# schmrlng/MotionPlanning.jl

Hardware: AMD Instinct MI355X
Metric: edges checked/sec + r-disc queries/sec, FMT* N=1e6 R^6, 1/2/4/8 MI355X (higher is better)
Workload: dtype f64

## Files before the change

### motionplanning.jl_amd/csrc/kernels_order.hip

```cpp
#include "mpfmt_internal.h"
#include <algorithm>

#define ORD_ID(k) ((k) & 0x03ffffffu)
#define ORD_COL(k) (((k) >> 26) & 15u)
#define ORD_THREADS 512
#define ORD_WAVES 8
#define ORD_COLS 16
#define ORD_NB 128
#define ORD_STG 2560
#define ORD_PRE 5
#define ORD_WAVES_EU 8
static_assert(ORD_STG >= MPFMT_ORD_MAXDEG, "a column the host lets through must fit the staging area");
static_assert(ORD_COLS * ORD_NB == ORD_THREADS * 4, "the segmented scan gives every thread four buckets");
static_assert(ORD_PRE * ORD_THREADS >= ORD_STG && ORD_STG % 32 == 0 && ORD_STG < 65536, "the prefetched records cover what the staging area holds; positions fit 16 bits");

struct ord_hdr {
    int32_t k[ORD_COLS];
    int32_t cb[ORD_COLS + 4];
    long long out[ORD_COLS];
    int32_t ho[ORD_COLS];
    int32_t n, pad_[3];
};
struct ord_shared {
    uint32_t cnt[ORD_COLS][ORD_NB / 2];
    uint32_t cur[ORD_COLS][ORD_NB / 2];
    ord_hdr h[2];
    int32_t g1, pcount, nextk, pad_;
    uint32_t bits[ORD_STG / 32];
};

__device__ __forceinline__ void lds_barrier()
{
    asm volatile("s_waitcnt lgkmcnt(0)\n\ts_barrier" ::: "memory");
}

struct ord_args {
    const uint32_t* qkey;
    const double* qd2;
    long long qcap;
    const int32_t* qlen;
    const int64_t* degs;
    int64_t tile_begin, tile_end;
    const int64_t* colptr;
    const int32_t* perm;
    const int32_t* iperm;
    int32_t* rowval;
    double* nzval;
    int32_t* rowpos;
    uint32_t bucket_mul;
    const int32_t* spec_fail;
    unsigned long long* mask;
    const int64_t* nnz_dev;
    uint4* pend_items; int64_t pend_wcap; int32_t* pend_cnt; int32_t* pend_over;
    int64_t* deg_clear;
    int rec_bits;
    int32_t* qctr;
};

__global__ __launch_bounds__(ORD_THREADS) __attribute__((amdgpu_waves_per_eu(ORD_WAVES_EU, ORD_WAVES_EU))) void k_order_logs(ord_args a)
{
    if (a.spec_fail && *a.spec_fail) return;
    extern __shared__ __attribute__((aligned(16))) char ord_smem[];
    double* const stage_d2 = reinterpret_cast<double*>(ord_smem);
    uint32_t* const stage_key = reinterpret_cast<uint32_t*>(ord_smem + ORD_STG * 8);
    ord_shared& sh = *reinterpret_cast<ord_shared*>(ord_smem + ORD_STG * 12);
    const int tid = threadIdx.x, lane = tid & 63;
    const int wave = __builtin_amdgcn_readfirstlane(tid >> 6);
    const int64_t nq = (a.tile_end - a.tile_begin) * 4;
    auto bucket = [&](uint32_t id) -> int { return a.bucket_mul ? min(ORD_NB - 1, (int)__umulhi(id, a.bucket_mul)) : (int)(id & (ORD_NB - 1)); };
    if (a.rec_bits && blockIdx.x == 0 && tid == 0) {
        const int64_t nnz = *a.nnz_dev;
        if (nnz & 63) atomicAnd(&a.mask[nnz >> 6], (1ull << (nnz & 63)) - 1ull);
    }

    int hk = 0, ho = -1, hln = 0;
    long long hout = 0;
    auto hdr_fetch1 = [&](int64_t qi) {
        hk = 0; ho = -1; hln = 0;
        if (qi >= nq) return;
        if (tid < ORD_COLS) {
            const int64_t sp = a.tile_begin * 64 + qi * ORD_COLS + tid;
            ho = a.perm[sp];
            hk = (int)a.degs[sp];
            if (a.deg_clear && ho >= 0) a.deg_clear[ho] = 0;
        } else if (tid == 64) {
            hln = (int)min((long long)a.qlen[qi], a.qcap);
        }
    };
    auto hdr_fetch2 = [&]() { hout = (tid < ORD_COLS && ho >= 0) ? a.colptr[ho] : 0; };
    auto hdr_publish = [&](int hb) {
        ord_hdr& H = sh.h[hb];
        if (tid < 64) {
            const int k = (tid < ORD_COLS && ho >= 0) ? hk : 0;
            int inc = k;
            inc += __builtin_amdgcn_update_dpp(0, inc, 0x111, 0xf, 0xf, true);
            inc += __builtin_amdgcn_update_dpp(0, inc, 0x112, 0xf, 0xf, true);
            inc += __builtin_amdgcn_update_dpp(0, inc, 0x114, 0xf, 0xf, true);
            inc += __builtin_amdgcn_update_dpp(0, inc, 0x118, 0xf, 0xf, true);
            if (tid < ORD_COLS) { H.k[tid] = k; H.cb[tid + 1] = inc; H.ho[tid] = ho; }
            if (tid == 0) H.cb[0] = 0;
        } else if (tid == 64) {
            H.n = hln;
        }
    };
    uint32_t pk[ORD_PRE];
    double pd[ORD_PRE];
    auto rec_fetch_n = [&](int total, int64_t qi) {
        const __amdgpu_buffer_rsrc_t rk = __builtin_amdgcn_make_buffer_rsrc(const_cast<uint32_t*>(a.qkey + (qi < nq ? qi : 0) * a.qcap), 0, total * 4, 0x00020000);
#pragma unroll
        for (int u = 0; u < ORD_PRE; ++u) pk[u] = __builtin_amdgcn_raw_buffer_load_b32(rk, tid * 4, u * ORD_THREADS * 4, 0);
    };
    auto rec_fetch = [&](const ord_hdr& H, int64_t qi) { rec_fetch_n((qi < nq) ? H.n : 0, qi); };
    typedef uint32_t ord_u32x2 __attribute__((ext_vector_type(2)));
    auto d2_fetch = [&](int total, int64_t qi) {
        const long long base = (qi < nq ? qi : 0) * a.qcap;
        const __amdgpu_buffer_rsrc_t rd = __builtin_amdgcn_make_buffer_rsrc(const_cast<double*>(a.qd2 + base), 0, total * 8, 0x00020000);
#pragma unroll
        for (int u = 0; u < ORD_PRE; ++u) {
            const ord_u32x2 v = __builtin_amdgcn_raw_buffer_load_b64(rd, tid * 8, u * ORD_THREADS * 8, 0);
            pd[u] = __hiloint2double((int)v.y, (int)v.x);
        }
    };

    if (tid == 0) sh.pcount = 0;
    int64_t qi = blockIdx.x;
    int64_t qn = qi + gridDim.x;
    const int xcd = (int)(blockIdx.x & 7u);
    int hb = 0;
    hdr_fetch1(qi);
    hdr_fetch2();
    hdr_publish(0);
    if (tid < ORD_COLS) sh.h[0].out[tid] = hout;
    lds_barrier();
    rec_fetch(sh.h[0], qi);
    d2_fetch(sh.h[0].n, qi);
    for (; qi < nq; hb ^= 1) {
        const ord_hdr& H = sh.h[hb];
        const int total = H.n;
        const long long lbase = qi * a.qcap;
        hdr_fetch1(qn);
            int g0 = 0;
        bool first = true;
        while (g0 < ORD_COLS) {
            if (tid < 64) {
                const bool ok = tid >= g0 && tid < ORD_COLS && (H.cb[min(tid, ORD_COLS - 1) + 1] - H.cb[g0] <= ORD_STG);
                const unsigned long long m = __ballot(ok);
                if (tid == 0) sh.g1 = g0 + (int)__popcll(m);
            }
            *reinterpret_cast<uint2*>(&sh.cnt[0][tid * 2]) = make_uint2(0u, 0u);
            lds_barrier();
            int g1 = sh.g1;
            const bool skip = g1 == g0;
            if (skip) g1 = g0 + 1;
            const int gb = H.cb[g0];
            auto for_records = [&](auto&& f) {
                if (first) {
#pragma unroll
                    for (int u = 0; u < ORD_PRE; ++u) if (u * ORD_THREADS + tid < total) {
                        uint32_t key = pk[u];
                        asm volatile("" : "+v"(key));
                        f(key, u, u * ORD_THREADS + tid);
                    }
                }
                for (int i = (first ? ORD_PRE * ORD_THREADS : 0) + tid; i < total; i += ORD_THREADS) f(a.qkey[lbase + i], -1, i);
            };
            if (!skip) for_records([&](uint32_t key, int, int) {
                const int col = (int)ORD_COL(key);
                if (col >= g0 && col < g1) { const int bk = bucket(ORD_ID(key)); atomicAdd(&sh.cnt[col][bk >> 1], 1u << ((bk & 1) * 16)); }
            });
            lds_barrier();
            {
                const int col = tid >> 5;
                const uint2 cw = *reinterpret_cast<const uint2*>(&sh.cnt[0][tid * 2]);
                const int c0 = (int)(cw.x & 0xffffu), c1 = (int)(cw.x >> 16), c2 = (int)(cw.y & 0xffffu), c3 = (int)(cw.y >> 16);
                const int tot = c0 + c1 + c2 + c3;
                int inc = tot;
                inc += __builtin_amdgcn_update_dpp(0, inc, 0x111, 0xf, 0xf, true);
                inc += __builtin_amdgcn_update_dpp(0, inc, 0x112, 0xf, 0xf, true);
                inc += __builtin_amdgcn_update_dpp(0, inc, 0x114, 0xf, 0xf, true);
                inc += __builtin_amdgcn_update_dpp(0, inc, 0x118, 0xf, 0xf, true);
                inc += __builtin_amdgcn_update_dpp(0, inc, 0x142, 0xa, 0xf, false);
                const int b0 = min(max(H.cb[col] - gb + inc - tot, 0), ORD_STG);
                const int b1 = min(b0 + c0, ORD_STG), b2 = min(b1 + c1, ORD_STG), b3 = min(b2 + c2, ORD_STG);
                *reinterpret_cast<uint2*>(&sh.cur[0][tid * 2]) = make_uint2((uint32_t)b0 | ((uint32_t)b1 << 16), (uint32_t)b2 | ((uint32_t)b3 << 16));
            }
            lds_barrier();
            if (!skip) for_records([&](uint32_t key, int u, int i) {
                const int col = (int)ORD_COL(key);
                if (col >= g0 && col < g1) {
                    const int bk = bucket(ORD_ID(key));
                    const int pos = (int)((atomicAdd(&sh.cur[col][bk >> 1], 1u << ((bk & 1) * 16)) >> ((bk & 1) * 16)) & 0xffffu);
                    double d2 = 0.0;
                    if (u < 0) d2 = a.qd2[lbase + i];
#pragma unroll
                    for (int v = 0; v < ORD_PRE; ++v) if (u == v) d2 = pd[v];
                    if (pos >= 0 && pos < ORD_STG) { stage_key[pos] = key; stage_d2[pos] = d2; }
                }
            });
            if (a.rec_bits && tid < ORD_STG / 32) sh.bits[tid] = 0xffffffffu;
            lds_barrier();
            if (first) {
                hdr_fetch2();
                hdr_publish(hb ^ 1);
                if (a.qctr && tid == 0) sh.nextk = atomicAdd(&a.qctr[xcd], 1);
                first = false;
            }
            const bool last_range = g1 >= ORD_COLS;
            if (last_range) {
                lds_barrier();
                rec_fetch(sh.h[hb ^ 1], qn);
                d2_fetch(qn < nq ? sh.h[hb ^ 1].n : 0, qn);
            }
            if (!skip) {
                const int nst = min(H.cb[g1] - gb, ORD_STG);
                for (int p0 = 0; p0 < nst; p0 += ORD_THREADS) {
                    const int p = p0 + tid;
                    const bool act = p < nst;
                    if (p0 + wave * 64 >= nst) break;
                    const uint32_t key = act ? stage_key[p] : ((uint32_t)(g1 - 1) << 26);
                    const int col = (int)ORD_COL(key);
                    const uint32_t id = ORD_ID(key);
                    const int bk = bucket(id);
                    const int e = (int)((sh.cur[col][bk >> 1] >> ((bk & 1) * 16)) & 0xffffu), n = (int)((sh.cnt[col][bk >> 1] >> ((bk & 1) * 16)) & 0xffffu);
                    int rk = e - n;
                    if (act) {
                        const int b0 = e - n, bl = e - 1;
                        const uint32_t m0 = ORD_ID(stage_key[b0]), m1 = ORD_ID(stage_key[min(b0 + 1, bl)]), m2 = ORD_ID(stage_key[min(b0 + 2, bl)]),
                                       m3 = ORD_ID(stage_key[min(b0 + 3, bl)]);
                        rk += (int)(m0 < id) + (int)(n > 1 && m1 < id) + (int)(n > 2 && m2 < id) + (int)(n > 3 && m3 < id);
                        for (int m = b0 + 4; m < e; ++m) rk += (ORD_ID(stage_key[m]) < id) ? 1 : 0;
                    }
                    const int rel = rk - (H.cb[col] - gb);
                    const bool valid = act && rel >= 0 && rel < H.k[col];
                    const int64_t o = H.out[col] + rel;
                    int32_t rp = 0;
                    const bool pd_ = valid && a.pend_items && ((key >> 30) & 1u);
                    if ((valid && a.rowpos) || pd_) rp = a.iperm[id];
                    if (valid) {
                        a.rowval[o] = (int32_t)id;
                        a.nzval[o] = sqrt(stage_d2[p]);
                        if (a.rowpos) a.rowpos[o] = rp;
                    }
                    if (a.rec_bits && valid && (key >> 31)) atomicAnd(&sh.bits[rk >> 5], ~(1u << (rk & 31)));
                    if (a.pend_items) {
                        const unsigned long long pm = __ballot(pd_);
                        if (pm) {
                            int base = 0;
                            if (lane == 0) base = atomicAdd(&sh.pcount, (int)__popcll(pm));
                            base = __builtin_amdgcn_readfirstlane(base);
                            if (pd_) {
                                const int pos = base + (int)__builtin_amdgcn_mbcnt_hi((uint32_t)(pm >> 32), __builtin_amdgcn_mbcnt_lo((uint32_t)pm, 0u));
                                if (pos < a.pend_wcap)
                                    a.pend_items[(int64_t)blockIdx.x * a.pend_wcap + pos] =
                                        make_uint4((uint32_t)(uint64_t)o, (uint32_t)((uint64_t)o >> 32), (uint32_t)H.ho[col], (uint32_t)rp);
                            }
                        }
                    }
                }
            }
            lds_barrier();
            if (a.rec_bits) {
                if (!skip) for (int c = g0 + 2 * wave; c < min(g1, g0 + 2 * wave + 2); ++c) {
                    const int k = H.k[c];
                    if (k == 0) continue;
                    const int sb = H.cb[c] - gb;
                    const int64_t o = H.out[c];
                    const int64_t w0 = o >> 6;
                    const int nw = (int)(((o + k - 1) >> 6) - w0) + 1;
                    for (int i = lane; i < nw; i += 64) {
                        const int64_t wd = w0 + i;
                        const int64_t lo_bit = max(wd * 64, o), hi_bit = min(wd * 64 + 64, o + k);
                        const int nb = (int)(hi_bit - lo_bit);
                        const int src = sb + (int)(lo_bit - o);
                        const int wi = src >> 5, sh5 = src & 31;
                        const unsigned long long a0 = sh.bits[wi], a1 = sh.bits[min(wi + 1, ORD_STG / 32 - 1)], a2 = sh.bits[min(wi + 2, ORD_STG / 32 - 1)];
                        unsigned long long val = (a0 | (a1 << 32)) >> sh5;
                        if (sh5) val |= a2 << (64 - sh5);
                        const unsigned long long keep = (nb == 64) ? ~0ull : ((1ull << nb) - 1ull);
                        const int dsh = (int)(lo_bit & 63);
                        const unsigned long long rng = keep << dsh;
                        const unsigned long long w64 = ((val & keep) << dsh) | ~rng;
                        if (w64 != ~0ull) atomicAnd(&a.mask[wd], w64);
                    }
                }
                lds_barrier();
            }
            g0 = g1;
        }
        if (tid < ORD_COLS) sh.h[hb ^ 1].out[tid] = hout;
        qi = qn;
        qn = a.qctr ? 2 * (int64_t)gridDim.x + xcd + 8 * (int64_t)sh.nextk : qn + gridDim.x;
    }
    if (a.pend_items) {
        lds_barrier();
        if (tid == 0) {
            const int c = sh.pcount;
            a.pend_cnt[blockIdx.x] = (int32_t)min((int64_t)c, a.pend_wcap);
            if (c > a.pend_wcap) *a.pend_over = 1;
        }
    }
}

int32_t mpfmt_mask_preset(mpfmt_ctx* ctx, int64_t entries)
{
    int32_t rc;
    const int64_t words = (entries + 63) / 64;
    if ((rc = ctx->graph_free.ensure(ctx, sizeof(uint64_t) * (size_t)(words + 1)))) return rc;
    HIPCHK(ctx, hipMemsetAsync(ctx->graph_free, 0xFF, sizeof(uint64_t) * (size_t)std::max<int64_t>(words, 1), ctx->stream));
    ctx->mask_preset_words = words;
    return MPFMT_OK;
}

int32_t mpfmt_order_logs(mpfmt_ctx* ctx, const int32_t* spec_fail, int64_t mask_entries)
{
    const int64_t nt = ctx->tile_end - ctx->tile_begin;
    int32_t rc;
    ctx->rowpos_valid = false;
    const bool recbits = ctx->bits_in_records;
    const bool pend = ctx->broad_in_drain && !recbits;
    if (recbits) {
        const int64_t words = (std::max<int64_t>(ctx->nnz, mask_entries) + 63) / 64;
        const int64_t words_alloc = (std::max<int64_t>((int64_t)((double)ctx->nnz * 1.02) + 4096, mask_entries) + 63) / 64 + 1;
        if ((rc = ctx->graph_free.ensure(ctx, sizeof(uint64_t) * (size_t)words_alloc))) return rc;
        if (!(ctx->mask_preset_words == words && ctx->nnz > 0))
            HIPCHK(ctx, hipMemsetAsync(ctx->graph_free, ctx->nnz > 0 ? 0xFF : 0, sizeof(uint64_t) * (size_t)std::max<int64_t>(words, 1), ctx->stream));
    }
    ctx->mask_preset_words = -1;
    if (ctx->nnz == 0 || nt <= 0) { if ((rc = mpfmt_side_join(ctx))) return rc; if (recbits) { ctx->graph_swept = true; ctx->sweep_in_order = true; } return MPFMT_OK; }
    const bool want_rowpos = !pend && !recbits;
    if (want_rowpos && (rc = ctx->rowpos.ensure(ctx, sizeof(int32_t) * (size_t)std::max<int64_t>(std::max(ctx->nnz, ctx->nnz_cap), 1)))) return rc;
    const size_t lds = (size_t)ORD_STG * 12 + sizeof(ord_shared);
    HIPCHK(ctx, hipFuncSetAttribute((const void*)k_order_logs, hipFuncAttributeMaxDynamicSharedMemorySize, (int)lds));
    if (ctx->ord_per_cu == 0) {
        int per_cu = 0;
        HIPCHK(ctx, hipOccupancyMaxActiveBlocksPerMultiprocessor(&per_cu, k_order_logs, ORD_THREADS, lds));
        ctx->ord_per_cu = std::max(1, std::min(per_cu, 4));
    }
    unsigned nb = (unsigned)std::min<int64_t>(nt * 4, (int64_t)ctx->num_cus * ctx->ord_per_cu);
    const bool draw = ctx->ord_draw && ctx->ord_ctr && nb >= 8 && (ctx->ord_draw > 1 || ctx->nnz >= (int64_t)1536 * nt * 4);
    if (draw) nb &= ~3u;
    if (pend) {
        const int64_t entries = std::max<int64_t>(ctx->nnz, ctx->nnz_cap);
        ctx->pend_wcap = ctx->debug_small_lists ? 8 : entries * 3 / (2 * (int64_t)nb) + 4096;
        if ((rc = ctx->pend_items.ensure(ctx, sizeof(uint4) * (size_t)ctx->pend_wcap * nb))) return rc;
        if ((rc = ctx->pend_cnt.ensure(ctx, sizeof(int32_t) * (size_t)(nb + 1)))) return rc;
        ctx->pend_over = ctx->pend_cnt + nb;
        HIPCHK(ctx, hipMemsetAsync(ctx->pend_over, 0, sizeof(int32_t), ctx->stream));
    }
    ord_args a{};
    a.qkey = ctx->qkey; a.qd2 = ctx->qd2; a.qcap = ctx->qcap; a.qlen = ctx->qlen; a.degs = ctx->degs;
    a.tile_begin = ctx->tile_begin; a.tile_end = ctx->tile_end; a.colptr = ctx->colptr; a.perm = ctx->perm; a.iperm = ctx->iperm;
    a.rowval = ctx->rowval; a.nzval = ctx->nzval; a.rowpos = want_rowpos ? ctx->rowpos : nullptr;
    a.bucket_mul = ctx->N > 128 ? (uint32_t)((128ull << 32) / (uint64_t)ctx->N) : 0u;
    a.spec_fail = spec_fail;
    a.mask = (unsigned long long*)ctx->graph_free.get(); a.nnz_dev = ctx->colptr + ctx->N;
    a.pend_items = pend ? (uint4*)ctx->pend_items.get() : nullptr; a.pend_wcap = ctx->pend_wcap; a.pend_cnt = ctx->pend_cnt; a.pend_over = ctx->pend_over;
    a.rec_bits = recbits ? 1 : 0;
    a.deg_clear = ctx->world > 1 ? ctx->deg : nullptr;
    a.qctr = draw ? ctx->ord_ctr : nullptr;
    if ((rc = mpfmt_side_join(ctx))) return rc;
    hipLaunchKernelGGL(k_order_logs, dim3(nb), dim3(ORD_THREADS), lds, ctx->stream, a);
    HIPCHK(ctx, hipGetLastError());
    if (pend) ctx->pend_nseg = (int)nb;
    ctx->pend_valid = pend;
    ctx->rowpos_valid = want_rowpos;
    if (recbits) { ctx->graph_swept = true; ctx->sweep_in_order = true; }
    return MPFMT_OK;
}
```

Baseline: 31.07 billion.

## Deepen order-kernel header pipeline to three stages and prefetch keys earlier

```diff
diff --git a/motionplanning.jl_amd/csrc/kernels_order.hip b/motionplanning.jl_amd/csrc/kernels_order.hip
--- a/motionplanning.jl_amd/csrc/kernels_order.hip
+++ b/motionplanning.jl_amd/csrc/kernels_order.hip
@@ -1,5 +1,7 @@
 #include "mpfmt_internal.h"
 #include <algorithm>
+#include <cstdio>
+#include <cstdlib>
 
 #define ORD_ID(k) ((k) & 0x03ffffffu)
 #define ORD_COL(k) (((k) >> 26) & 15u)
@@ -9,6 +11,7 @@
 #define ORD_NB 128
 #define ORD_STG 2560
 #define ORD_PRE 5
+#define ORD_CLK_N 12
 #define ORD_WAVES_EU 8
 static_assert(ORD_STG >= MPFMT_ORD_MAXDEG, "a column the host lets through must fit the staging area");
 static_assert(ORD_COLS * ORD_NB == ORD_THREADS * 4, "the segmented scan gives every thread four buckets");
@@ -24,15 +27,28 @@
 struct ord_shared {
     uint32_t cnt[ORD_COLS][ORD_NB / 2];
     uint32_t cur[ORD_COLS][ORD_NB / 2];
-    ord_hdr h[2];
+    ord_hdr h[3];
     int32_t g1, pcount, nextk, pad_;
     uint32_t bits[ORD_STG / 32];
+#ifdef ORD_CLOCK
+    unsigned long long clk[ORD_CLK_N];
+#endif
 };
+static_assert(ORD_STG * 12 + sizeof(ord_shared) <= 40960, "four workgroups per CU: a quarter of the CU's 160 KB of LDS each");
 
 __device__ __forceinline__ void lds_barrier()
 {
     asm volatile("s_waitcnt lgkmcnt(0)\n\ts_barrier" ::: "memory");
 }
+
+#ifdef ORD_CLOCK
+__device__ unsigned long long ord_clk_dev[4096][ORD_CLK_N];
+#define ORD_CLK(i) do { if (wave == 0) { const unsigned long long t_ = __builtin_readcyclecounter(); if (lane == 0) atomicAdd(&sh.clk[i], t_ - clk_prev); clk_prev = t_; } } while (0)
+#define ORD_CLK_USE5(x) asm volatile("" :: "v"(x[0]), "v"(x[1]), "v"(x[2]), "v"(x[3]), "v"(x[4]))
+#else
+#define ORD_CLK(i) do {} while (0)
+#define ORD_CLK_USE5(x) do {} while (0)
+#endif
 
 struct ord_args {
     const uint32_t* qkey;
@@ -57,7 +73,7 @@
     int32_t* qctr;
 };
 
-__global__ __launch_bounds__(ORD_THREADS) __attribute__((amdgpu_waves_per_eu(ORD_WAVES_EU, ORD_WAVES_EU))) void k_order_logs(ord_args a)
+template <int MODE> __global__ __launch_bounds__(ORD_THREADS) __attribute__((amdgpu_waves_per_eu(ORD_WAVES_EU, ORD_WAVES_EU))) void k_order_logs(ord_args a)
 {
     if (a.spec_fail && *a.spec_fail) return;
     extern __shared__ __attribute__((aligned(16))) char ord_smem[];
@@ -68,51 +84,58 @@
     const int wave = __builtin_amdgcn_readfirstlane(tid >> 6);
     const int64_t nq = (a.tile_end - a.tile_begin) * 4;
     auto bucket = [&](uint32_t id) -> int { return a.bucket_mul ? min(ORD_NB - 1, (int)__umulhi(id, a.bucket_mul)) : (int)(id & (ORD_NB - 1)); };
-    if (a.rec_bits && blockIdx.x == 0 && tid == 0) {
+    constexpr bool REC_BITS = MODE == 2, PEND = MODE == 1, ROWPOS = MODE == 0;
+    if (REC_BITS && blockIdx.x == 0 && tid == 0) {
         const int64_t nnz = *a.nnz_dev;
         if (nnz & 63) atomicAnd(&a.mask[nnz >> 6], (1ull << (nnz & 63)) - 1ull);
     }
 
     int hk = 0, ho = -1, hln = 0;
     long long hout = 0;
-    auto hdr_fetch1 = [&](int64_t qi) {
-        hk = 0; ho = -1; hln = 0;
-        if (qi >= nq) return;
-        if (tid < ORD_COLS) {
-            const int64_t sp = a.tile_begin * 64 + qi * ORD_COLS + tid;
-            ho = a.perm[sp];
-            hk = (int)a.degs[sp];
-            if (a.deg_clear && ho >= 0) a.deg_clear[ho] = 0;
-        } else if (tid == 64) {
-            hln = (int)min((long long)a.qlen[qi], a.qcap);
+    auto hdr_fetch1 = [&](int64_t qi, int g) {
+        if ((tid >> 4) == g) {
+            hk = 0; ho = -1;
+            if (qi < nq) {
+                const int64_t sp = a.tile_begin * 64 + qi * ORD_COLS + (tid & 15);
+                ho = a.perm[sp];
+                hk = (int)a.degs[sp];
+                if (a.deg_clear && ho >= 0) a.deg_clear[ho] = 0;
+            }
+        } else if (tid == 64 + g) {
+            hln = (qi < nq) ? (int)min((long long)a.qlen[qi], a.qcap) : 0;
         }
     };
-    auto hdr_fetch2 = [&]() { hout = (tid < ORD_COLS && ho >= 0) ? a.colptr[ho] : 0; };
-    auto hdr_publish = [&](int hb) {
-        ord_hdr& H = sh.h[hb];
+    auto hdr_fetch2 = [&](int ng) { hout = (tid < ORD_COLS * ng && ho >= 0) ? a.colptr[ho] : 0; };
+    auto hdr_publish = [&](int s0, int ng) {
         if (tid < 64) {
-            const int k = (tid < ORD_COLS && ho >= 0) ? hk : 0;
+            const int g = tid >> 4, c = tid & 15;
+            const int k = (g < ng && ho >= 0) ? hk : 0;
             int inc = k;
             inc += __builtin_amdgcn_update_dpp(0, inc, 0x111, 0xf, 0xf, true);
             inc += __builtin_amdgcn_update_dpp(0, inc, 0x112, 0xf, 0xf, true);
             inc += __builtin_amdgcn_update_dpp(0, inc, 0x114, 0xf, 0xf, true);
             inc += __builtin_amdgcn_update_dpp(0, inc, 0x118, 0xf, 0xf, true);
-            if (tid < ORD_COLS) { H.k[tid] = k; H.cb[tid + 1] = inc; H.ho[tid] = ho; }
-            if (tid == 0) H.cb[0] = 0;
-        } else if (tid == 64) {
-            H.n = hln;
+            if (g < ng) {
+                ord_hdr& H = sh.h[s0 + g];
+                H.k[c] = k; H.cb[c + 1] = inc; H.ho[c] = ho;
+                if (c == 0) H.cb[0] = 0;
+            }
+        } else if (tid < 64 + ng) {
+            sh.h[s0 + tid - 64].n = hln;
         }
     };
-    uint32_t pk[ORD_PRE];
+    auto hdr_out = [&](int s0, int ng) { if (tid < ORD_COLS * ng) sh.h[s0 + (tid >> 4)].out[tid & 15] = hout; };
+    uint32_t pk[ORD_PRE], rk[ORD_PRE];
     double pd[ORD_PRE];
-    auto rec_fetch_n = [&](int total, int64_t qi) {
-        const __amdgpu_buffer_rsrc_t rk = __builtin_amdgcn_make_buffer_rsrc(const_cast<uint32_t*>(a.qkey + (qi < nq ? qi : 0) * a.qcap), 0, total * 4, 0x00020000);
+    auto key_fetch = [&](uint32_t (&k)[ORD_PRE], int total, int64_t qi) {
+        total = __builtin_amdgcn_readfirstlane(total);
+        const __amdgpu_buffer_rsrc_t rs = __builtin_amdgcn_make_buffer_rsrc(const_cast<uint32_t*>(a.qkey + (qi < nq ? qi : 0) * a.qcap), 0, total * 4, 0x00020000);
 #pragma unroll
-        for (int u = 0; u < ORD_PRE; ++u) pk[u] = __builtin_amdgcn_raw_buffer_load_b32(rk, tid * 4, u * ORD_THREADS * 4, 0);
+        for (int u = 0; u < ORD_PRE; ++u) k[u] = __builtin_amdgcn_raw_buffer_load_b32(rs, tid * 4, u * ORD_THREADS * 4, 0);
     };
-    auto rec_fetch = [&](const ord_hdr& H, int64_t qi) { rec_fetch_n((qi < nq) ? H.n : 0, qi); };
     typedef uint32_t ord_u32x2 __attribute__((ext_vector_type(2)));
     auto d2_fetch = [&](int total, int64_t qi) {
+        total = __builtin_amdgcn_readfirstlane(total);
         const long long base = (qi < nq ? qi : 0) * a.qcap;
         const __amdgpu_buffer_rsrc_t rd = __builtin_amdgcn_make_buffer_rsrc(const_cast<double*>(a.qd2 + base), 0, total * 8, 0x00020000);
 #pragma unroll
@@ -126,20 +149,31 @@
     int64_t qi = blockIdx.x;
     int64_t qn = qi + gridDim.x;
     const int xcd = (int)(blockIdx.x & 7u);
-    int hb = 0;
-    hdr_fetch1(qi);
-    hdr_fetch2();
-    hdr_publish(0);
-    if (tid < ORD_COLS) sh.h[0].out[tid] = hout;
+    int drawn = 0;
+    if (a.qctr && tid == 0) drawn = atomicAdd(&a.qctr[xcd], 1);
+    hdr_fetch1(qi, 0);
+    hdr_fetch1(qn, 1);
+    hdr_fetch2(2);
+    hdr_publish(0, 2);
+    hdr_out(0, 2);
+    if (tid == 0) sh.nextk = drawn;
+#ifdef ORD_CLOCK
+    if (tid < ORD_CLK_N) sh.clk[tid] = 0;
+    unsigned long long clk_prev = __builtin_readcyclecounter();
+    const unsigned long long clk_begin = clk_prev;
+#endif
     lds_barrier();
-    rec_fetch(sh.h[0], qi);
+    int64_t qn2 = a.qctr ? 2 * (int64_t)gridDim.x + xcd + 8 * (int64_t)__builtin_amdgcn_readfirstlane(sh.nextk) : qn + gridDim.x;
+    key_fetch(pk, sh.h[0].n, qi);
     d2_fetch(sh.h[0].n, qi);
-    for (; qi < nq; hb ^= 1) {
-        const ord_hdr& H = sh.h[hb];
+    for (int hs = 0; qi < nq; hs = (hs == 2) ? 0 : hs + 1) {
+        const int hs1 = (hs == 2) ? 0 : hs + 1, hs2 = (hs1 == 2) ? 0 : hs1 + 1;
+        const ord_hdr& H = sh.h[hs];
         const int total = H.n;
         const long long lbase = qi * a.qcap;
-        hdr_fetch1(qn);
-            int g0 = 0;
+        ORD_CLK(9);
+        hdr_fetch1(qn2, 0);
+        int g0 = 0;
         bool first = true;
         while (g0 < ORD_COLS) {
             if (tid < 64) {
@@ -153,22 +187,30 @@
             const bool skip = g1 == g0;
             if (skip) g1 = g0 + 1;
             const int gb = H.cb[g0];
-            auto for_records = [&](auto&& f) {
+            auto for_records = [&](const uint32_t (&kk)[ORD_PRE], auto&& f) {
                 if (first) {
 #pragma unroll
                     for (int u = 0; u < ORD_PRE; ++u) if (u * ORD_THREADS + tid < total) {
-                        uint32_t key = pk[u];
+                        uint32_t key = kk[u];
                         asm volatile("" : "+v"(key));
                         f(key, u, u * ORD_THREADS + tid);
                     }
                 }
                 for (int i = (first ? ORD_PRE * ORD_THREADS : 0) + tid; i < total; i += ORD_THREADS) f(a.qkey[lbase + i], -1, i);
             };
-            if (!skip) for_records([&](uint32_t key, int, int) {
+            ORD_CLK(0);
+            if (first) ORD_CLK_USE5(pk);
+            ORD_CLK(1);
+            if (!skip) for_records(pk, [&](uint32_t key, int, int) {
                 const int col = (int)ORD_COL(key);
                 if (col >= g0 && col < g1) { const int bk = bucket(ORD_ID(key)); atomicAdd(&sh.cnt[col][bk >> 1], 1u << ((bk & 1) * 16)); }
             });
+            if (first) {
+                key_fetch(rk, total, qi);
+                key_fetch(pk, (qn < nq) ? sh.h[hs1].n : 0, qn);
+            }
             lds_barrier();
+            ORD_CLK(2);
             {
                 const int col = tid >> 5;
                 const uint2 cw = *reinterpret_cast<const uint2*>(&sh.cnt[0][tid * 2]);
@@ -185,7 +227,10 @@
                 *reinterpret_cast<uint2*>(&sh.cur[0][tid * 2]) = make_uint2((uint32_t)b0 | ((uint32_t)b1 << 16), (uint32_t)b2 | ((uint32_t)b3 << 16));
             }
             lds_barrier();
-            if (!skip) for_records([&](uint32_t key, int u, int i) {
+            ORD_CLK(3);
+            if (first) { ORD_CLK_USE5(rk); ORD_CLK_USE5(pd); }
+            ORD_CLK(4);
+            if (!skip) for_records(rk, [&](uint32_t key, int u, int i) {
                 const int col = (int)ORD_COL(key);
                 if (col >= g0 && col < g1) {
                     const int bk = bucket(ORD_ID(key));
@@ -197,20 +242,18 @@
                     if (pos >= 0 && pos < ORD_STG) { stage_key[pos] = key; stage_d2[pos] = d2; }
                 }
             });
-            if (a.rec_bits && tid < ORD_STG / 32) sh.bits[tid] = 0xffffffffu;
+            if (REC_BITS && tid < ORD_STG / 32) sh.bits[tid] = 0xffffffffu;
             lds_barrier();
+            ORD_CLK(5);
             if (first) {
-                hdr_fetch2();
-                hdr_publish(hb ^ 1);
+                hdr_fetch2(1);
+                hdr_publish(hs2, 1);
                 if (a.qctr && tid == 0) sh.nextk = atomicAdd(&a.qctr[xcd], 1);
                 first = false;
             }
             const bool last_range = g1 >= ORD_COLS;
-            if (last_range) {
-                lds_barrier();
-                rec_fetch(sh.h[hb ^ 1], qn);
-                d2_fetch(qn < nq ? sh.h[hb ^ 1].n : 0, qn);
-            }
+            if (last_range) d2_fetch(qn < nq ? sh.h[hs1].n : 0, qn);
+            ORD_CLK(6);
             if (!skip) {
                 const int nst = min(H.cb[g1] - gb, ORD_STG);
                 for (int p0 = 0; p0 < nst; p0 += ORD_THREADS) {
@@ -222,27 +265,27 @@
                     const uint32_t id = ORD_ID(key);
                     const int bk = bucket(id);
                     const int e = (int)((sh.cur[col][bk >> 1] >> ((bk & 1) * 16)) & 0xffffu), n = (int)((sh.cnt[col][bk >> 1] >> ((bk & 1) * 16)) & 0xffffu);
-                    int rk = e - n;
+                    int rnk = e - n;
                     if (act) {
                         const int b0 = e - n, bl = e - 1;
                         const uint32_t m0 = ORD_ID(stage_key[b0]), m1 = ORD_ID(stage_key[min(b0 + 1, bl)]), m2 = ORD_ID(stage_key[min(b0 + 2, bl)]),
                                        m3 = ORD_ID(stage_key[min(b0 + 3, bl)]);
-                        rk += (int)(m0 < id) + (int)(n > 1 && m1 < id) + (int)(n > 2 && m2 < id) + (int)(n > 3 && m3 < id);
-                        for (int m = b0 + 4; m < e; ++m) rk += (ORD_ID(stage_key[m]) < id) ? 1 : 0;
+                        rnk += (int)(m0 < id) + (int)(n > 1 && m1 < id) + (int)(n > 2 && m2 < id) + (int)(n > 3 && m3 < id);
+                        for (int m = b0 + 4; m < e; ++m) rnk += (ORD_ID(stage_key[m]) < id) ? 1 : 0;
                     }
-                    const int rel = rk - (H.cb[col] - gb);
+                    const int rel = rnk - (H.cb[col] - gb);
                     const bool valid = act && rel >= 0 && rel < H.k[col];
                     const int64_t o = H.out[col] + rel;
                     int32_t rp = 0;
-                    const bool pd_ = valid && a.pend_items && ((key >> 30) & 1u);
-                    if ((valid && a.rowpos) || pd_) rp = a.iperm[id];
+                    const bool pd_ = valid && PEND && ((key >> 30) & 1u);
+                    if ((valid && ROWPOS) || pd_) rp = a.iperm[id];
                     if (valid) {
                         a.rowval[o] = (int32_t)id;
                         a.nzval[o] = sqrt(stage_d2[p]);
-                        if (a.rowpos) a.rowpos[o] = rp;
+                        if (ROWPOS) a.rowpos[o] = rp;
                     }
-                    if (a.rec_bits && valid && (key >> 31)) atomicAnd(&sh.bits[rk >> 5], ~(1u << (rk & 31)));
-                    if (a.pend_items) {
+                    if (REC_BITS && valid && (key >> 31)) atomicAnd(&sh.bits[rnk >> 5], ~(1u << (rnk & 31)));
+                    if (PEND) {
                         const unsigned long long pm = __ballot(pd_);
                         if (pm) {
                             int base = 0;
@@ -259,7 +302,8 @@
                 }
             }
             lds_barrier();
-            if (a.rec_bits) {
+            ORD_CLK(7);
+            if (REC_BITS) {
                 if (!skip) for (int c = g0 + 2 * wave; c < min(g1, g0 + 2 * wave + 2); ++c) {
                     const int k = H.k[c];
                     if (k == 0) continue;
@@ -284,14 +328,23 @@
                     }
                 }
                 lds_barrier();
+                ORD_CLK(8);
             }
             g0 = g1;
         }
-        if (tid < ORD_COLS) sh.h[hb ^ 1].out[tid] = hout;
+        hdr_out(hs2, 1);
         qi = qn;
-        qn = a.qctr ? 2 * (int64_t)gridDim.x + xcd + 8 * (int64_t)sh.nextk : qn + gridDim.x;
-    }
-    if (a.pend_items) {
+        qn = qn2;
+        qn2 = a.qctr ? 2 * (int64_t)gridDim.x + xcd + 8 * (int64_t)__builtin_amdgcn_readfirstlane(sh.nextk) : qn2 + gridDim.x;
+#ifdef ORD_CLOCK
+        if (tid == 0) atomicAdd(&sh.clk[10], 1ull);
+#endif
+    }
+#ifdef ORD_CLOCK
+    lds_barrier();
+    if (tid < ORD_CLK_N && blockIdx.x < 4096) ord_clk_dev[blockIdx.x][tid] = (tid == 11) ? __builtin_readcyclecounter() - clk_begin : sh.clk[tid];
+#endif
+    if (PEND) {
         lds_barrier();
         if (tid == 0) {
             const int c = sh.pcount;
@@ -330,10 +383,11 @@
     const bool want_rowpos = !pend && !recbits;
     if (want_rowpos && (rc = ctx->rowpos.ensure(ctx, sizeof(int32_t) * (size_t)std::max<int64_t>(std::max(ctx->nnz, ctx->nnz_cap), 1)))) return rc;
     const size_t lds = (size_t)ORD_STG * 12 + sizeof(ord_shared);
-    HIPCHK(ctx, hipFuncSetAttribute((const void*)k_order_logs, hipFuncAttributeMaxDynamicSharedMemorySize, (int)lds));
+    const auto kern = recbits ? k_order_logs<2> : (pend ? k_order_logs<1> : k_order_logs<0>);
+    HIPCHK(ctx, hipFuncSetAttribute((const void*)kern, hipFuncAttributeMaxDynamicSharedMemorySize, (int)lds));
     if (ctx->ord_per_cu == 0) {
         int per_cu = 0;
-        HIPCHK(ctx, hipOccupancyMaxActiveBlocksPerMultiprocessor(&per_cu, k_order_logs, ORD_THREADS, lds));
+        HIPCHK(ctx, hipOccupancyMaxActiveBlocksPerMultiprocessor(&per_cu, kern, ORD_THREADS, lds));
         ctx->ord_per_cu = std::max(1, std::min(per_cu, 4));
     }
     unsigned nb = (unsigned)std::min<int64_t>(nt * 4, (int64_t)ctx->num_cus * ctx->ord_per_cu);
@@ -359,8 +413,29 @@
     a.deg_clear = ctx->world > 1 ? ctx->deg : nullptr;
     a.qctr = draw ? ctx->ord_ctr : nullptr;
     if ((rc = mpfmt_side_join(ctx))) return rc;
-    hipLaunchKernelGGL(k_order_logs, dim3(nb), dim3(ORD_THREADS), lds, ctx->stream, a);
+    hipLaunchKernelGGL(kern, dim3(nb), dim3(ORD_THREADS), lds, ctx->stream, a);
     HIPCHK(ctx, hipGetLastError());
+#ifdef ORD_CLOCK
+    if (const char* path = getenv("MPFMT_ORD_CLOCK_OUT")) {
+        static unsigned long long rows[4096][ORD_CLK_N];
+        static double sum[ORD_CLK_N], launches;
+        HIPCHK(ctx, hipStreamSynchronize(ctx->stream));
+        HIPCHK(ctx, hipMemcpyFromSymbol(rows, HIP_SYMBOL(ord_clk_dev), sizeof(rows)));
+        for (unsigned b = 0; b < std::min(nb, 4096u); ++b) for (int i = 0; i < ORD_CLK_N; ++i) sum[i] += (double)rows[b][i];
+        launches += 1;
+        if (FILE* f = fopen(path, "w")) {
+            static const char* nm[ORD_CLK_N] = {"range setup", "wait: keys (COUNT's first use)", "COUNT", "scan", "wait: d2 and PLACE's keys", "PLACE",
+                                                "header publish, draw, requests", "WRITE", "mask bits", "tail", "quarters", "kernel"};
+            double tot = 0;
+            for (int i = 0; i < 10; ++i) tot += sum[i];
+            fprintf(f, "launches %.0f  workgroups %u  quarters per launch %.0f  device-clock ticks per workgroup and launch %.0f\n", launches, nb, sum[10] / launches, sum[11] / launches / nb);
+            fprintf(f, "%-34s %14s %8s\n", "interval", "ticks/quarter", "share");
+            for (int i = 0; i < 10; ++i) fprintf(f, "%-34s %14.1f %7.1f%%\n", nm[i], sum[i] / sum[10], 100.0 * sum[i] / tot);
+            fprintf(f, "%-34s %14.1f\n", "sum", tot / sum[10]);
+            fclose(f);
+        }
+    }
+#endif
     if (pend) ctx->pend_nseg = (int)nb;
     ctx->pend_valid = pend;
     ctx->rowpos_valid = want_rowpos;
```

Result: no change. 31.09 billion, median of 2 (+0.1%).
